# Bebra777228/PolGen-RVC

Measured on AMD Instinct MI355X. Metric: real-time-factor (audio-sec/wall-sec) per GPU, 30s@16kHz RMVPE->48kHz, higher is better.
Workload: dtype f32 (conv products as 3 fp16 MFMAs of a hi/lo split, fp32 accumulate; fp32 elsewhere)

## Files before the change

### include/rvcx.h

```cpp
#ifndef RVCX_H
#define RVCX_H
#include <stdint.h>

#ifdef __cplusplus
extern "C" {
#endif

typedef struct rvcx_ctx rvcx_ctx;

typedef struct {
  const char* name;
  const void* data;
  int32_t dtype;
  int32_t ndim;
  int64_t shape[4];
} rvcx_tensor;

typedef struct {
  int32_t inter_channels, hidden_channels, filter_channels, n_heads, n_layers, kernel_size;
  int32_t n_resblocks;
  int32_t res_kernels[4];
  int32_t res_dilations[4][3];
  int32_t n_ups;
  int32_t up_rates[6], up_kernels[6];
// ... 359 lines not shown
int rvcx_debug_inject(rvcx_ctx*, int what);
double rvcx_flop_counter(rvcx_ctx*, int reset);
void* rvcx_stream(rvcx_ctx*);

int rvcx_op_fcpe_post(rvcx_ctx*, const float* raw_hd, int F_in, int p_len, double pitch, double f0_min, double f0_max,
                      int32_t* coarse, float* f0);
int rvcx_op_conv1d(rvcx_ctx*, const float* x, const float* w, const float* bias, const float* res,
                   float* y, int B, int Cin, int Tin, int Cout, int K, int stride, int dil,
                   int pad_left, int Tout, int groups, int pre_lrelu, float pre_slope, int act,
                   float act_slope, const int32_t* lens_in, const int32_t* lens_out);
int rvcx_op_resblock_pair(rvcx_ctx*, const float* x, const float* w1, const float* b1, const float* w2,
                          const float* b2, float* y, int B, int C, int T, int K, int dil, float slope, int fused,
                          const int32_t* lens);
int rvcx_op_resblock3(rvcx_ctx*, const float* x, const float* w1, const float* b1, const float* w2, const float* b2,
                      float* y, int B, int C, int T, const int32_t* dils, float slope, const int32_t* lens);
int rvcx_bench_resblock_pair(rvcx_ctx*, int B, int C, int T, int K, int dil, int fused, int iters,
                             float* ms_per_launch);
int rvcx_bench_conv1d(rvcx_ctx*, int B, int Cin, int Tin, int Cout, int K, int stride, int dil, int groups,
                      int iters, float* ms_per_launch);
int rvcx_conv_override(int tile, int variant, int splitk);
int rvcx_fx_stretch_override(int chunk_frames, int segment_frames);
int rvcx_op_convtranspose1d(rvcx_ctx*, const float* x, const float* w, const float* bias, float* y,
                            int B, int Cin, int Tin, int Cout, int K, int stride, int pad,
                            int pre_lrelu, float pre_slope);
int rvcx_op_conv2d3x3(rvcx_ctx*, const float* x, const float* w, const float* bias, const float* res,
                      float* y, int B, int Cin, int H, int W, int Cout, int act);
int rvcx_op_convblock2d(rvcx_ctx*, const float* x, const float* w1, const float* b1, const float* w2, const float* b2,
                        const float* wsc, const float* bsc, float* y, int B, int Cin, int Cout, int H, int W,
                        const int32_t* rows);
int rvcx_op_convtranspose2d(rvcx_ctx*, const float* x, const float* w, const float* bias, float* y,
// ... 44 lines not shown
```

### polgen-rvc_amd/_lib.py

```python
from __future__ import annotations

import ctypes as C
import os
import threading
import types
from typing import Optional, Sequence

import numpy as np

_HERE = os.path.dirname(os.path.abspath(__file__))
LIB_PATH = os.environ.get("RVCX_LIBRARY") or os.path.join(_HERE, "librvcx.so")


class RvcxError(RuntimeError):
    pass


class Tensor(C.Structure):
    _fields_ = [("name", C.c_char_p), ("data", C.c_void_p), ("dtype", C.c_int32),
                ("ndim", C.c_int32), ("shape", C.c_int64 * 4)]


class SynthCfg(C.Structure):
    _fields_ = [("inter_channels", C.c_int32), ("hidden_channels", C.c_int32),
# ... 98 lines not shown
    k = min(Lx, Lb)
    fin = np.sin(0.5 * np.pi * np.arange(Lx) / max(Lx - 1, 1)) ** 2
    out[:k] = y[d:d + k] * fin[:k] + b[:k] * (1.0 - fin[:k])
    return out, y[d + Lb:d + Lb + Lx].copy(), d, scores, mags


_lib = None

SYMBOLS = [
    "rvcx_create", "rvcx_destroy", "rvcx_last_error", "rvcx_version", "rvcx_load_hubert",
    "rvcx_load_rmvpe", "rvcx_index_exhaustive", "rvcx_load_crepe", "rvcx_crepe_frames", "rvcx_crepe_predict", "rvcx_op_crepe_decode", "rvcx_get_f0_crepe_x", "rvcx_load_fcpe", "rvcx_fcpe_f0", "rvcx_fcpe_frames", "rvcx_get_f0_fcpe_x", "rvcx_op_fcpe_post", "rvcx_load_synth", "rvcx_unload_synth", "rvcx_load_index", "rvcx_load_index_ivf",
    "rvcx_weights_regions", "rvcx_weights_adopt", "rvcx_weights_clone", "rvcx_rmvpe_f0", "rvcx_rmvpe_frames", "rvcx_rmvpe_mel", "rvcx_synth_infer_taps", "rvcx_hubert_features",
    "rvcx_hubert_frames", "rvcx_synth_infer", "rvcx_synth_infer_window", "rvcx_synth_dec_rf", "rvcx_synth_upp", "rvcx_index_blend",
    "rvcx_out_len", "rvcx_convert_batch", "rvcx_convert_batch_f64", "rvcx_micro_batch", "rvcx_bucket_length", "rvcx_last_micro_batches", "rvcx_last_cuts", "rvcx_noise_len",
    "rvcx_get_f0", "rvcx_get_f0_x", "rvcx_vc", "rvcx_vc_frames", "rvcx_last_timing",
    "rvcx_flop_counter", "rvcx_fp32_reruns", "rvcx_mem_info", "rvcx_conv_profile", "rvcx_conv_profile_csv", "rvcx_stream", "rvcx_op_conv1d", "rvcx_op_resblock_pair", "rvcx_bench_resblock_pair", "rvcx_bench_conv1d", "rvcx_conv_override", "rvcx_op_convtranspose1d",
    "rvcx_op_conv2d3x3", "rvcx_op_convblock2d", "rvcx_op_convtranspose2d", "rvcx_op_attention", "rvcx_op_layernorm_c",
    "rvcx_op_bigru", "rvcx_op_highpass", "rvcx_highpass_exact", "rvcx_convert_batch_ex", "rvcx_get_f0_x_ex", "rvcx_fp32_layers", "rvcx_fp32_pinned",
    "rvcx_gru_fallbacks", "rvcx_gru_publish_probe", "rvcx_debug_inject", "rvcx_f0_file_track", "rvcx_op_gemm_tm", "rvcx_op_layernorm_tm",
    "rvcx_resample_len", "rvcx_resample_f64", "rvcx_resample_f64_kind", "rvcx_bench_gemm", "rvcx_device_info",
    "rvcx_convert_submit", "rvcx_convert_wait", "rvcx_convert_poll", "rvcx_convert_inflight", "rvcx_ticket_lead_ms",
    "rvcx_synth_infer_head", "rvcx_op_sola", "rvcx_stream_open", "rvcx_stream_step", "rvcx_stream_reset", "rvcx_stream_close",
    "rvcx_stream_out_len", "rvcx_stream_noise_len", "rvcx_stream_frames",
    "rvcx_stream_open_io", "rvcx_stream_in_len", "rvcx_stream_delays", "rvcx_stream_resample_delay", "rvcx_stream_last_taps",
    "rvcx_stream_set", "rvcx_op_stream_resample",
    "rvcx_stream_open_fx", "rvcx_stream_out_channels", "rvcx_stream_set_fx", "rvcx_stream_last_fx_ms", "rvcx_op_stream_fx",
    "rvcx_fx_reverb_host",
    "rvcx_fx_chain", "rvcx_op_fx_highpass", "rvcx_op_fx_compressor", "rvcx_op_fx_gate", "rvcx_op_fx_reverb", "rvcx_op_fx_shelf",
    "rvcx_op_fx_chorus", "rvcx_op_fx_mix", "rvcx_fx_chunk", "rvcx_fx_last_passes", "rvcx_fx_cte", "rvcx_fx_delay",
    "rvcx_fx_coeffs", "rvcx_fx_highpass_host", "rvcx_fx_biquad_host", "rvcx_fx_follower_host", "rvcx_fx_compressor_host",
    "rvcx_fx_gate_host", "rvcx_fx_comb_host", "rvcx_fx_allpass_host", "rvcx_fx_chorus_host", "rvcx_fx_mix_host",
# ... 1006 lines not shown
        return y

    def resblock_pair(self, x, w1, b1, w2, b2, dil=1, slope=0.1, fused=True, lens=None):
        x, w1, w2 = f32(x), f32(w1), f32(w2)
        B, Cc, T = x.shape
        K = w1.shape[2]
        y = np.empty_like(x)
        b1 = None if b1 is None else f32(b1)
        b2 = None if b2 is None else f32(b2)
        li = i32(lens)
        self._ck(lib().rvcx_op_resblock_pair(self._h, _p(x), _p(w1), _p(b1), _p(w2), _p(b2), _p(y), B, Cc, T, K, dil,
                                             C.c_float(slope), 1 if fused else 0, _p(li, C.c_int32)),
                 "op_resblock_pair")
        return y

    def resblock3(self, x, w1, b1, w2, b2, dils=(1, 3, 5), slope=0.1, lens=None):
        x, w1, w2 = f32(x), f32(w1), f32(w2)
        B, Cc, T = x.shape
        y = np.empty_like(x)
        b1 = None if b1 is None else f32(b1)
        b2 = None if b2 is None else f32(b2)
        d = i32(list(dils))
        li = i32(lens)
        self._ck(lib().rvcx_op_resblock3(self._h, _p(x), _p(w1), _p(b1), _p(w2), _p(b2), _p(y), B, Cc, T, _p(d, C.c_int32),
                                         C.c_float(slope), _p(li, C.c_int32)), "op_resblock3")
        return y

    def bench_resblock_pair(self, B, Cc, T, K, dil=1, fused=True, iters=10):
        ms = C.c_float(0)
        self._ck(lib().rvcx_bench_resblock_pair(self._h, B, Cc, T, K, dil, 1 if fused else 0, iters, C.byref(ms)),
# ... 1088 lines not shown
```

### polgen-rvc_amd/csrc/api_ops.hip

```cpp
#include "api_internal.h"
#include "h3_device.h"

using namespace rvcx;
using namespace rvcx::api;

static void to_host(Ctx& c, float* h, const float* d, size_t n) {
  RVCX_HIP(hipMemcpyAsync(h, d, n * sizeof(float), hipMemcpyDeviceToHost, c.stream));
  RVCX_HIP(hipStreamSynchronize(c.stream));
}
#define TEMP_REGION(C) WeightRegion tmp_region_; RegionScope tmp_scope_(*(C), tmp_region_)

extern "C" {

int rvcx_op_conv1d(rvcx_ctx* ctx, const float* x, const float* w, const float* bias, const float* res,
                   float* y, int B, int Cin, int Tin, int Cout, int K, int stride, int dil,
                   int pad_left, int Tout, int groups, int pre_lrelu, float pre_slope, int act,
                   float act_slope, const int32_t* lens_in, const int32_t* lens_out) {
  API_BEGIN(ctx)
  TEMP_REGION(C);
  size_t nx = (size_t)B * Cin * Tin, ny = (size_t)B * Cout * Tout;
  C->arena.reserve((nx + 2 * ny) * 4 + (64 << 20));
  C->arena.reset();
  ConvW L = make_conv(*C, w, bias, Cout, Cin / groups, K, groups, true);
  float* dx = to_dev(*C, x, nx);
// ... 211 lines not shown
  RVCX_HIP(hipEventCreate(&e0));
  RVCX_HIP(hipEventCreate(&e1));
  RVCX_HIP(hipEventRecord(e0, C->stream));
  for (int i = 0; i < iters; ++i) once();
  RVCX_HIP(hipEventRecord(e1, C->stream));
  RVCX_HIP(hipEventSynchronize(e1));
  float ms = 0.f;
  RVCX_HIP(hipEventElapsedTime(&ms, e0, e1));
  *ms_per_launch = ms / iters;
  (void)hipEventDestroy(e0);
  (void)hipEventDestroy(e1);
  C->arena.reset();
  API_END
}

int rvcx_conv_override(int tile, int variant, int splitk) {
  REQUIRE_DEBUG(nullptr, "rvcx_conv_override")
  rvcx::g_conv_override.tile = tile;
  rvcx::g_conv_override.variant = variant;
  rvcx::g_conv_override.splitk = splitk;
  return 0;
}

int rvcx_bench_conv1d(rvcx_ctx* ctx, int B, int Cin, int Tin, int Cout, int K, int stride, int dil, int groups,
                      int iters, float* ms_per_launch) {
  REQUIRE_DEBUG(ctx, "rvcx_bench_conv1d")
  API_BEGIN(ctx)
  TEMP_REGION(C);
  const int pad = (K * dil - dil) / 2;
  const int Tout = (Tin + 2 * pad - dil * (K - 1) - 1) / stride + 1;
// ... 660 lines not shown
```

### polgen-rvc_amd/csrc/conv.h

```cpp
#pragma once
#include "common.h"

namespace rvcx {

enum Act { ACT_NONE = 0, ACT_LRELU = 1, ACT_RELU = 2, ACT_GELU = 3, ACT_TANH = 4, ACT_SIGMOID = 5 };
enum OutMode { OUT_NORMAL = 0, OUT_SHUF1D = 1, OUT_SHUF2D = 2, OUT_TRANSPOSED = 3 };
enum Acc2 { ACC2_NONE = 0, ACC2_SET = 1, ACC2_ADD = 2, ACC2_ADD_DIV = 3 };

struct ConvArgs {
  const float* x = nullptr;
  const float* w = nullptr;
  const void* w_h3 = nullptr;
  const void* x_split = nullptr;
  void* y_split = nullptr;
  const float* bias = nullptr;
  const float* res = nullptr;
  float* y = nullptr;
  float* y2 = nullptr;
  const int* lens_in = nullptr;
  const int* lens_out = nullptr;
  int B = 1;
  int Cin_g = 0, Cin_gp = 0, Cout_g = 0, Cout_gp = 0, groups = 1;
  int Tin = 0;
  int Nout = 0;
// ... 117 lines not shown
bool convt_thin_ok(const ConvArgs& a);
void launch_convt_thin(const ConvArgs& a, hipStream_t stream);
void convt_thin_init();
constexpr int kConvtThinSlot = 61;
bool conv3_thin_ok(const ConvArgs& a);
void launch_conv3_thin(const ConvArgs& a, hipStream_t stream);
constexpr int kConv3ThinSlot = 59;
bool conv_deep_ok(const ConvArgs& a);
void launch_conv_deep(const ConvArgs& a, hipStream_t stream);
constexpr int kConvDeepSlot = 63;
bool conv_h3_enabled();
bool conv_h3_configured();
bool conv_h3_split_ok(const ConvArgs& a);
void launch_splitk_finish(const ConvArgs& a, hipStream_t stream);
void conv_h3_describe(ConvProfile* p);
struct ConvOverride { int tile = -1, variant = -1, splitk = -1; };
extern ConvOverride g_conv_override;
void conv_fast_init();
double conv_flops(const ConvArgs& a);

int conv_cin_pad(int cin_g);
int conv_cout_pad(int cout_g);
std::vector<float> pack_conv_weight(const float* w, int cout, int cin_g, int k, int groups);
struct PolyPhase1d {
  std::vector<float> w;
  std::vector<float> bias;
  int taps = 0;
  int pad = 0;
  int cout_total = 0;
};
// ... 5 lines not shown
```

### polgen-rvc_amd/csrc/conv_h3.hip

```cpp
#include <algorithm>
#include <cmath>
#include <cstdlib>

#include "conv.h"
#include "conv_device.h"
#include "h3_device.h"

#ifdef RVCX_ABLATION
#define H3_DBG(a, bit) ((a).dbg & (bit))
#else
#define H3_DBG(a, bit) 0
#endif

namespace rvcx {

template <int BM, int BN, int WR, int WC, int KKT, int HALO, int STRIDE, bool LIN, bool XS = false>
__global__ __launch_bounds__(256, ((LIN && BM * BN >= 8192) || BN >= 512) ? 2 : 3) void conv_h3_kernel(const ConvArgs a) {
  constexpr int WM = BM / (32 * WR), WN = BN / (32 * WC);
  constexpr int WROW = LIN ? BN : BN * STRIDE + HALO;
  constexpr int NBTILE = LIN ? KKT : 1;
  constexpr int A_ELEMS = KKT * 2 * 2 * BM;
  constexpr int NA = (A_ELEMS + 255) / 256;
  constexpr int B_TASKS = NBTILE * 2 * WROW;
  constexpr int NBT = (B_TASKS + 255) / 256;
// ... 310 lines not shown
  if (a.groups != 1 || a.ksize == 1 || a.out_mode != OUT_NORMAL) return false;
  if (a.stride != 1 && !(a.stride == 2 && a.kw == a.ksize)) return false;
  if (a.Cin_g % 16 != 0 || a.Cout_g % 16 != 0 || a.Cin_g != a.Cin_gp) return false;
  {
    int lo = 1 << 30, hi = -(1 << 30);
    for (int kk = 0; kk < a.ksize; ++kk) {
      lo = std::min(lo, conv_tap_off(a, kk));
      hi = std::max(hi, conv_tap_off(a, kk));
    }
    if (hi - lo > 320) return false;
  }
  if ((long)a.Cin_gp * a.x_cs * 4 >= kH3Oob || (long)a.Cout_g * a.y_cs * 4 >= kH3Oob) return false;
  return true;
}

int launch_conv_h3(ConvArgs& a, int halo, int off_min, hipStream_t stream) {
  const bool split = a.x_split || a.y_split;
  RVCX_CHECK(!split || conv_h3_split_ok(a), "conv_h3: pre-split activations on a launch that cannot take them");
  if (!a.w_h3 || !conv_h3_enabled()) return -1;
  if (a.Cin_gp % 16 != 0 || (a.stride != 1 && !(a.stride == 2 && a.kw == a.ksize))) return -1;
  if (a.groups != 1 && (split || a.ksize == 1 || a.stride != 1 || a.out_mode != OUT_NORMAL || a.Cin_g != a.Cin_gp)) return -1;
  if ((long)a.Cin_gp * a.x_cs * 4 >= kH3Oob || (long)a.ksize * a.Cin_gp * a.Cout_gp * 4 >= kH3Oob) return -1;
  const bool lin = a.ksize == 1 && a.stride == 1;
  const int nchunk = a.Cin_gp / 16;
  const long cap_item = a.part_cap_item > 0 ? a.part_cap_item : a.part_cap;
  static const bool wide3x3 = getenv("RVCX_WIDE3X3") && atoi(getenv("RVCX_WIDE3X3")) != 0;
  auto select = [&](int Bsel, int forcedS, int* tile_out, int* s_out) {
    int best = -1, S = 1;
    double best_t = 1e300;
    for (int t = 0; t < kNumH3; ++t) {
      const H3Cfg& F = kH3[t];
      if (g_conv_override.tile >= 100 && g_conv_override.tile - 100 != t) continue;
      if (F.lin != lin || F.stride != a.stride) continue;
// ... 22 lines not shown
    *tile_out = best;
    *s_out = S;
  };
  int best = -1, S = 1;
  select(1, 0, &best, &S);
  static const int tile2_mask = getenv("RVCX_TILE2_MASK") ? atoi(getenv("RVCX_TILE2_MASK")) : 255;
  const int cls = (a.out_mode != OUT_NORMAL) ? 8 : (lin ? 2 : (halo > 64 ? 1 : 4));
  int cls2 = cls;
  if (a.x_split || a.y_split) cls2 |= 16;
  const bool tile_for_batch = (tile2_mask & cls) && (!(cls2 & 16) || (tile2_mask & 16));
  if (best >= 0 && a.B > 1 && tile_for_batch) {
    int b2 = -1, s2 = 1;
    select(a.B, S, &b2, &s2);
    if (b2 >= 0 && s2 == S) best = b2;
  }
  if (best < 0) return -1;
  const H3Cfg& F = kH3[best];
  a.off_min = off_min;
  a.wrow = halo;
  a.splitk = S;
  {
    static int dbg = -1;
    if (dbg < 0) dbg = getenv("RVCX_CONV_DBG") ? atoi(getenv("RVCX_CONV_DBG")) : 0;
    a.dbg = dbg;
  }
  dim3 grid(cdiv(a.Nout, F.bn), cdiv(a.Cout_gp, F.bm), a.B * a.groups * S);
  {
    static const bool log = getenv("RVCX_CONV_LOG") != nullptr;
    if (log)
      fprintf(stderr, "h3 tile %d (%dx%d halo %d) S %d grid %u %u %u B %d Cin %d Cout %d k %d Nout %d xs %d ys %d\n", best,
              F.bm, F.bn, F.halo, S, grid.x, grid.y, grid.z, a.B, a.Cin_g, a.Cout_g, a.ksize, a.Nout, a.x_split != nullptr,
              a.y_split != nullptr);
  }
  hipLaunchKernelGGL(a.x_split ? F.kern_xs : F.kern, grid, dim3(256), 0, stream, a);
  if (S > 1) launch_splitk_finish(a, stream);
  RVCX_HIP(hipGetLastError());
  return h3_slot(best);
}

}
```

### polgen-rvc_amd/csrc/ctx.h

```cpp
#pragma once
#include <memory>

#include "common.h"
#include "conv.h"
#include "gemm.h"

namespace rvcx {

struct SynthModel;
struct RmvpeModel;
struct FcpeModel;
struct CrepeModel;
struct HubertModel;
struct IndexData;

class WeightRegion {
 public:
  static constexpr size_t kChunkBytes = (size_t)32 << 20;
  static constexpr int kMaxFlags = 4096;
  static constexpr size_t kHeaderBytes = kMaxFlags;
  WeightRegion() {
    flags_.reset(new uint8_t[kMaxFlags]);
    std::memset(flags_.get(), 0, kMaxFlags);
  }
// ... 224 lines not shown
  }
  void gemm_on(GemmArgs a, hipStream_t s) {
    const double f = 2.0 * (double)a.rows * a.cout * a.cin;
    flops += f;
    a.ovf = dev_err;
    a.seq = ++launch_seq;
    {
      const int si = (s == stream2) ? 1 : (s == aux[0] ? 2 : (s == aux[1] ? 3 : 0));
      if (!splitk_buf[si]) RVCX_HIP(hipMalloc(&splitk_buf[si], kSplitKFloats * splitk_items * sizeof(float)));
      a.part = splitk_buf[si];
      a.part_cap = kSplitKFloats * splitk_items;
    }
    conv_launch_gemm(a, f, s);
  }
  void conv(const ConvArgs& a) { conv_on(a, stream); }
  void conv_on(ConvArgs a, hipStream_t s) {
    flops += conv_flops(a);
    const int si = (s == stream2) ? 1 : (s == aux[0] ? 2 : (s == aux[1] ? 3 : 0));
    if (!splitk_buf[si]) RVCX_HIP(hipMalloc(&splitk_buf[si], kSplitKFloats * splitk_items * sizeof(float)));
    a.part = splitk_buf[si];
    a.part_cap = kSplitKFloats * splitk_items;
    a.part_cap_item = kSplitKFloats;
    a.ovf = dev_err;
    a.seq = ++launch_seq;
    launch_conv(a, s);
  }
};

struct RegionScope {
  Ctx& c;
  WeightRegion* prev;
  RegionScope(Ctx& cc, WeightRegion& r) : c(cc), prev(cc.slab.cur_) { cc.slab.cur_ = &r; }
  ~RegionScope() { c.slab.cur_ = prev; }
};

struct ConvW {
  const float* w = nullptr;
// ... 56 lines not shown
```

### polgen-rvc_amd/csrc/layers.h

```cpp
#pragma once
#include "ctx.h"

namespace rvcx {

inline ConvArgs conv1d_args(const ConvW& w, const float* x, float* y, int B, int Tin, int Tout,
                            int stride = 1, int dil = 1, int pad = 0) {
  ConvArgs a;
  conv_set_weights(a, w);
  a.x = x;
  a.y = y;
  a.B = B;
  a.Tin = Tin;
  a.Nout = Tout;
  a.stride = stride;
  a.dil = dil;
  a.pad = pad;
  a.x_bs = (long)w.cin * Tin;
  a.x_cs = Tin;
  a.y_bs = (long)w.cout * Tout;
  a.y_cs = Tout;
  return a;
}

inline void conv_set_res(ConvArgs& a, const float* res, int C, int T) {
  a.res = res;
  a.res_bs = (long)C * T;
  a.res_cs = T;
}

struct ConvT1dW {
  ConvW w;
  int stride = 1, pad_t = 0, cout_real = 0, k_orig = 0, taps_pad = 0;
};

inline ConvArgs convT1d_args(const ConvT1dW& L, const float* x, float* y, int B, int Tin, int Tout) {
  ConvArgs a;
  conv_set_weights(a, L.w);
  a.x = x;
  a.y = y;
  a.B = B;
  a.Tin = Tin;
  a.Nout = cdiv(Tout + L.pad_t, L.stride);
  a.stride = 1;
// ... 76 lines not shown
```

### polgen-rvc_amd/csrc/ops.hip

```cpp
#include <algorithm>
#include <cmath>
#include <vector>

#include "conv.h"
#include "h3_device.h"
#include "ops.h"

namespace rvcx {

__device__ __forceinline__ float wave_sum(float v) {
#pragma unroll
  for (int o = 32; o > 0; o >>= 1) v += __shfl_xor(v, o);
  return v;
}

__device__ __forceinline__ float gelu_erf(float v) {
  return 0.5f * v * (1.f + erff(v * 0.70710678118654752440f));
}

constexpr int LN_TX = 16, LN_PARTS = 16, LN_MAXC = 1024, LN_RPT = LN_MAXC / LN_PARTS;
__global__ __launch_bounds__(256) void layernorm_c_kernel(const float* __restrict__ x,
                                                          const float* __restrict__ gamma,
                                                          const float* __restrict__ beta, float* __restrict__ y,
                                                          int C, int T, float eps, const int* lens) {
// ... 475 lines not shown
}
void launch_flip_channels(const float* x, float* y, int B, int C, int T, hipStream_t s) {
  long n = (long)B * C * T;
  hipLaunchKernelGGL(flip_channels_kernel, EW_GRID(n), 0, s, x, y, C, T, n);
}

__global__ void wn_gate_kernel(const float* a, const float* g, int goff, int gstride, float* acts, int H, int T,
                               long total) {
  for (long idx = blockIdx.x * 256L + threadIdx.x; idx < total; idx += (long)gridDim.x * 256) {
    const int t = idx % T;
    const long bc = idx / T;
    const int c = bc % H;
    const long b = bc / H;
    const float ta = a[(b * 2 * H + c) * T + t] + g[b * gstride + goff + c];
    const float sa = a[(b * 2 * H + H + c) * T + t] + g[b * gstride + goff + H + c];
    acts[idx] = tanhf(ta) * (1.f / (1.f + expf(-sa)));
  }
}
void launch_wn_gate(const float* a, const float* g, int goff, int gstride, float* acts, int B, int H, int T,
                    hipStream_t s) {
  long n = (long)B * H * T;
  hipLaunchKernelGGL(wn_gate_kernel, EW_GRID(n), 0, s, a, g, goff, gstride, acts, H, T, n);
}

__global__ void wn_res_skip_kernel(float* x, float* out, const float* rs, int H, int T, int last, int first,
                                   const int* lens, long total) {
  for (long idx = blockIdx.x * 256L + threadIdx.x; idx < total; idx += (long)gridDim.x * 256) {
    const int t = idx % T;
    const long bc = idx / T;
    const int c = bc % H;
    const long b = bc / H;
// ... 472 lines not shown
```

### polgen-rvc_amd/csrc/synth.hip

```cpp
#include <algorithm>
#include <cmath>
#include <cstdlib>

#include "models.h"
#include "ops.h"

namespace rvcx {

std::vector<float> wn_weight(const TensorTable& t, const std::string& p, int dim) {
  if (t.has(p + ".weight")) return t.f32(p + ".weight");
  std::string gn = p + ".parametrizations.weight.original0", vn = p + ".parametrizations.weight.original1";
  if (!t.has(gn)) {
    gn = p + ".weight_g";
    vn = p + ".weight_v";
  }
  std::vector<float> g = t.f32(gn), v = t.f32(vn);
  const auto shp = t.shape(vn);
  RVCX_CHECK(shp.size() == 3, "weight-norm tensor must be 3-D: " + p);
  const int64_t d0 = shp[0], d1 = shp[1], d2 = shp[2];
  std::vector<float> w(v.size());
  if (dim == 0) {
    RVCX_CHECK((int64_t)g.size() == d0, "weight_g shape: " + p);
    for (int64_t a = 0; a < d0; ++a) {
      double ss = 0.0;
// ... 312 lines not shown

  float* z = A.alloc<float>((size_t)B * inter * T);
  float* z2 = A.alloc<float>((size_t)B * inter * T);
  launch_sample_z(stats, io.z_noise, z, B, inter, T, lens, s);
  if (head > 0) {
    launch_copy_strided(z + head, z2, B * inter, Tk, T, Tk, s);
    std::swap(z, z2);
  }
  float* g = A.alloc<float>((size_t)B * gin);
  for (int b = 0; b < B; ++b)
    RVCX_HIP(hipMemcpyAsync(g + (size_t)b * gin, m.emb_g + (size_t)sidv[b] * gin, gin * sizeof(float),
                            hipMemcpyDeviceToDevice, s));
  {
    float* h = att;
    float* xin = qkv;
    float* acts = tmp;
    float* rs = hbuf;
    RVCX_CHECK(filt >= 2 * hid, "buffer reuse assumes filter_channels >= 2*hidden");
    float* wout = A.alloc<float>((size_t)B * hid * T);
    float* mbuf = A.alloc<float>((size_t)B * half * T);
    float* gc = A.alloc<float>((size_t)B * 6 * hid);
    for (int f = 3; f >= 0; --f) {
      const auto& F = m.flows[f];
      launch_flip_channels(z, z2, B, inter, Tk, s);
      std::swap(z, z2);
      ConvArgs a = conv1d_args(F.pre, z, h, B, Tk, Tk);
      a.x_bs = (long)inter * Tk;
      a.lens_out = lens;
      c.conv(a);
      a = conv1d_args(F.cond, g, gc, B, 1, 1);
      c.conv(a);
      for (int i = 0; i < 3; ++i) {
        a = conv1d_args(F.in_l[i], h, xin, B, Tk, Tk, 1, 1, (F.in_l[i].k - 1) / 2);
        a.lens_in = lens;
        a.lens_out = lens;
        c.conv(a);
        launch_wn_gate(xin, gc, i * 2 * hid, 6 * hid, acts, B, hid, Tk, s);
        a = conv1d_args(F.rs_l[i], acts, rs, B, Tk, Tk);
        a.lens_out = lens;
        c.conv(a);
        launch_wn_res_skip(h, wout, rs, B, hid, Tk, i == 2, i == 0, lens, s);
      }
      a = conv1d_args(F.post, wout, mbuf, B, Tk, Tk);
      a.lens_out = lens;
      c.conv(a);
      launch_coupling_sub(z, mbuf, B, half, Tk, lens, s);
    }
  }
  if (io.z_out)
    RVCX_HIP(hipMemcpyAsync(io.z_out, z, (size_t)B * inter * Tk * sizeof(float), hipMemcpyDeviceToDevice, s));
  tm.mark(2);
  if (io.ev_decoder) RVCX_HIP(hipEventRecord(io.ev_decoder, s));

  if (!c.serial) RVCX_HIP(hipStreamWaitEvent(s, c.ev_src[1], 0));
  static const int dec_batch_env = getenv("RVCX_DEC_BATCH") ? std::max(1, atoi(getenv("RVCX_DEC_BATCH"))) : 8;
  bool equal_lens = true;
// ... 207 lines not shown
```

Measured before the change: 1224.

## Fuse WaveNet flow layer into a single MFMA kernel

Adds a fused kernel for each WaveNet layer in the flow. It runs the K=5 input conv, the tanh·sigmoid gate, the 1x1 res/skip conv and the residual/skip accumulation in one launch, keeping the gated activations in shared memory as hi/lo fp16 splits. This replaces four launches per layer and the global-memory round-trips for xin, acts and rs. The cost is a specialized kernel limited to hid=192 and K=5, split-k handled by in-register folding, and a fallback to the old path for any other shape.

```diff
diff --git a/include/rvcx.h b/include/rvcx.h
--- a/include/rvcx.h
+++ b/include/rvcx.h
@@ -397,6 +397,10 @@
                           const int32_t* lens);
 int rvcx_op_resblock3(rvcx_ctx*, const float* x, const float* w1, const float* b1, const float* w2, const float* b2,
                       float* y, int B, int C, int T, const int32_t* dils, float slope, const int32_t* lens);
+int rvcx_op_wn_layer(rvcx_ctx*, const float* h, const float* wout, const float* gc, const float* w_in, const float* b_in,
+                     const float* w_rs, const float* b_rs, float* h_out, float* wout_out, int B, int hid, int T, int K, int goff,
+                     int gstride, int first, int last, int fused, const int32_t* lens);
+int rvcx_bench_wn_layer(rvcx_ctx*, int B, int T, int last, int fused, int iters, float* ms_per_layer);
 int rvcx_bench_resblock_pair(rvcx_ctx*, int B, int C, int T, int K, int dil, int fused, int iters,
                              float* ms_per_launch);
 int rvcx_bench_conv1d(rvcx_ctx*, int B, int Cin, int Tin, int Cout, int K, int stride, int dil, int groups,
diff --git a/polgen-rvc_amd/_lib.py b/polgen-rvc_amd/_lib.py
--- a/polgen-rvc_amd/_lib.py
+++ b/polgen-rvc_amd/_lib.py
@@ -136,7 +136,7 @@
     "rvcx_hubert_frames", "rvcx_synth_infer", "rvcx_synth_infer_window", "rvcx_synth_dec_rf", "rvcx_synth_upp", "rvcx_index_blend",
     "rvcx_out_len", "rvcx_convert_batch", "rvcx_convert_batch_f64", "rvcx_micro_batch", "rvcx_bucket_length", "rvcx_last_micro_batches", "rvcx_last_cuts", "rvcx_noise_len",
     "rvcx_get_f0", "rvcx_get_f0_x", "rvcx_vc", "rvcx_vc_frames", "rvcx_last_timing",
-    "rvcx_flop_counter", "rvcx_fp32_reruns", "rvcx_mem_info", "rvcx_conv_profile", "rvcx_conv_profile_csv", "rvcx_stream", "rvcx_op_conv1d", "rvcx_op_resblock_pair", "rvcx_bench_resblock_pair", "rvcx_bench_conv1d", "rvcx_conv_override", "rvcx_op_convtranspose1d",
+    "rvcx_flop_counter", "rvcx_fp32_reruns", "rvcx_mem_info", "rvcx_conv_profile", "rvcx_conv_profile_csv", "rvcx_stream", "rvcx_op_conv1d", "rvcx_op_resblock_pair", "rvcx_op_wn_layer", "rvcx_bench_wn_layer", "rvcx_bench_resblock_pair", "rvcx_bench_conv1d", "rvcx_conv_override", "rvcx_op_convtranspose1d",
     "rvcx_op_conv2d3x3", "rvcx_op_convblock2d", "rvcx_op_convtranspose2d", "rvcx_op_attention", "rvcx_op_layernorm_c",
     "rvcx_op_bigru", "rvcx_op_highpass", "rvcx_highpass_exact", "rvcx_convert_batch_ex", "rvcx_get_f0_x_ex", "rvcx_fp32_layers", "rvcx_fp32_pinned",
     "rvcx_gru_fallbacks", "rvcx_gru_publish_probe", "rvcx_debug_inject", "rvcx_f0_file_track", "rvcx_op_gemm_tm", "rvcx_op_layernorm_tm",
@@ -1173,6 +1173,24 @@
                  "op_resblock_pair")
         return y
 
+    def wn_layer(self, h, wout, gc, w_in, b_in, w_rs, b_rs, goff=0, first=False, last=False, fused=True, lens=None):
+        h, gc, w_in, w_rs, b_in, b_rs = f32(h), f32(gc), f32(w_in), f32(w_rs), f32(b_in), f32(b_rs)
+        B, hid, T = h.shape
+        wout = np.zeros_like(h) if wout is None else f32(wout)
+        h_out, wout_out = np.empty_like(h), np.empty_like(h)
+        li = i32(lens)
+        self._ck(lib().rvcx_op_wn_layer(self._h, _p(h), _p(wout), _p(gc), _p(w_in), _p(b_in), _p(w_rs), _p(b_rs),
+                                        _p(h_out), _p(wout_out), B, hid, T, w_in.shape[2], goff, gc.shape[1],
+                                        1 if first else 0, 1 if last else 0, 1 if fused else 0, _p(li, C.c_int32)),
+                 "op_wn_layer")
+        return h_out, wout_out
+
+    def bench_wn_layer(self, B, T, last=False, fused=True, iters=20):
+        ms = C.c_float(0)
+        self._ck(lib().rvcx_bench_wn_layer(self._h, B, T, 1 if last else 0, 1 if fused else 0, iters, C.byref(ms)),
+                 "bench_wn_layer")
+        return ms.value
+
     def resblock3(self, x, w1, b1, w2, b2, dils=(1, 3, 5), slope=0.1, lens=None):
         x, w1, w2 = f32(x), f32(w1), f32(w2)
         B, Cc, T = x.shape
diff --git a/polgen-rvc_amd/csrc/api_ops.hip b/polgen-rvc_amd/csrc/api_ops.hip
--- a/polgen-rvc_amd/csrc/api_ops.hip
+++ b/polgen-rvc_amd/csrc/api_ops.hip
@@ -249,6 +249,91 @@
   API_END
 }
 
+int rvcx_op_wn_layer(rvcx_ctx* ctx, const float* h, const float* wout, const float* gc, const float* w_in, const float* b_in,
+                     const float* w_rs, const float* b_rs, float* h_out, float* wout_out, int B, int hid, int T, int K, int goff,
+                     int gstride, int first, int last, int fused, const int32_t* lens) {
+  API_BEGIN(ctx)
+  TEMP_REGION(C);
+  const size_t n = (size_t)B * hid * T;
+  C->arena.reserve(n * 4 * 8 + (64 << 20));
+  C->arena.reset();
+  ConvW Li = make_conv(*C, w_in, b_in, 2 * hid, hid, K, 1, true);
+  ConvW Lr = make_conv(*C, w_rs, b_rs, last ? hid : 2 * hid, hid, 1, 1, true);
+  float* dh = to_dev(*C, h, n);
+  float* dalt = C->arena.alloc<float>(n);
+  float* dw = C->arena.alloc<float>(n);
+  if (first) RVCX_HIP(hipMemsetAsync(dw, 0xff, n * 4, C->stream));
+  else RVCX_HIP(hipMemcpyAsync(dw, wout, n * 4, hipMemcpyDefault, C->stream));
+  RVCX_HIP(hipMemsetAsync(dalt, 0xff, n * 4, C->stream));
+  float* dxin = C->arena.alloc<float>(2 * n);
+  float* drs = C->arena.alloc<float>(2 * n);
+  WnStep st;
+  st.in_l = &Li;
+  st.rs_l = &Lr;
+  st.gc = to_dev(*C, gc, (size_t)B * gstride);
+  st.goff = goff;
+  st.gstride = gstride;
+  st.lens = (lens ? to_dev(*C, lens, B) : nullptr);
+  st.B = B;
+  st.hid = hid;
+  st.T = T;
+  st.first = first;
+  st.last = last;
+  const float* dres = wn_layer_on(*C, st, dh, dalt, dw, dxin, drs, (fused && !g_force_fp32) ? 1 : 0);
+  to_host(*C, h_out, dres, n);
+  to_host(*C, wout_out, dw, n);
+  C->arena.reset();
+  API_END
+}
+
+int rvcx_bench_wn_layer(rvcx_ctx* ctx, int B, int T, int last, int fused, int iters, float* ms_per_layer) {
+  REQUIRE_DEBUG(ctx, "rvcx_bench_wn_layer")
+  API_BEGIN(ctx)
+  TEMP_REGION(C);
+  const int hid = 192, K = 5;
+  const size_t n = (size_t)B * hid * T;
+  C->arena.reserve(n * 4 * 8 + (64 << 20));
+  C->arena.reset();
+  std::vector<float> wi((size_t)2 * hid * hid * K), wr((size_t)2 * hid * hid), bias((size_t)2 * hid, 0.05f), g((size_t)B * 2 * hid, 0.1f);
+  for (size_t i = 0; i < wi.size(); ++i) wi[i] = ((float)((i * 2654435761u) % 2001) / 1000.f - 1.f) / std::sqrt((float)hid * K);
+  for (size_t i = 0; i < wr.size(); ++i) wr[i] = ((float)((i * 2246822519u) % 2001) / 1000.f - 1.f) / (4.f * std::sqrt((float)hid));
+  ConvW Li = make_conv(*C, wi.data(), bias.data(), 2 * hid, hid, K, 1, true);
+  ConvW Lr = make_conv(*C, wr.data(), bias.data(), last ? hid : 2 * hid, hid, 1, 1, true);
+  float* dh = C->arena.alloc<float>(n);
+  float* dalt = C->arena.alloc<float>(n);
+  float* dw = C->arena.alloc<float>(n);
+  float* dxin = C->arena.alloc<float>(2 * n);
+  float* drs = C->arena.alloc<float>(2 * n);
+  launch_randn(dh, n, 1, 0, C->stream);
+  RVCX_HIP(hipMemsetAsync(dw, 0, n * 4, C->stream));
+  WnStep st;
+  st.in_l = &Li;
+  st.rs_l = &Lr;
+  st.gc = to_dev(*C, g.data(), g.size());
+  st.gstride = 2 * hid;
+  st.B = B;
+  st.hid = hid;
+  st.T = T;
+  st.last = last;
+  RVCX_HIP(hipStreamSynchronize(C->stream));
+  auto once = [&]() { (void)wn_layer_on(*C, st, dh, dalt, dw, dxin, drs, fused ? 1 : 0); };
+  once();
+  hipEvent_t e0, e1;
+  RVCX_HIP(hipEventCreate(&e0));
+  RVCX_HIP(hipEventCreate(&e1));
+  RVCX_HIP(hipEventRecord(e0, C->stream));
+  for (int i = 0; i < iters; ++i) once();
+  RVCX_HIP(hipEventRecord(e1, C->stream));
+  RVCX_HIP(hipEventSynchronize(e1));
+  float ms = 0.f;
+  RVCX_HIP(hipEventElapsedTime(&ms, e0, e1));
+  *ms_per_layer = ms / iters;
+  (void)hipEventDestroy(e0);
+  (void)hipEventDestroy(e1);
+  C->arena.reset();
+  API_END
+}
+
 int rvcx_conv_override(int tile, int variant, int splitk) {
   REQUIRE_DEBUG(nullptr, "rvcx_conv_override")
   rvcx::g_conv_override.tile = tile;
diff --git a/polgen-rvc_amd/csrc/conv.h b/polgen-rvc_amd/csrc/conv.h
--- a/polgen-rvc_amd/csrc/conv.h
+++ b/polgen-rvc_amd/csrc/conv.h
@@ -155,6 +155,29 @@
 bool conv_h3_split_ok(const ConvArgs& a);
 void launch_splitk_finish(const ConvArgs& a, hipStream_t stream);
 void conv_h3_describe(ConvProfile* p);
+int conv_h3_splitk(const ConvArgs& a);
+
+struct WnArgs {
+  const float* h = nullptr;
+  float* h_out = nullptr;
+  float* wout = nullptr;
+  const float* gc = nullptr;
+  int goff = 0, gstride = 0;
+  const void* w_in = nullptr;
+  const void* w_rs = nullptr;
+  const float* b_in = nullptr;
+  const float* b_rs = nullptr;
+  const int* lens = nullptr;
+  int B = 1, hid = 0, k = 0, T = 0;
+  int first = 0, last = 0;
+  int splitk = 1;
+  int* ovf = nullptr;
+  int* ovf_in = nullptr;
+  int* ovf_rs = nullptr;
+  int seq = 0;
+};
+bool wn_layer_ok(const WnArgs& a);
+void launch_wn_layer(const WnArgs& a, hipStream_t stream);
 struct ConvOverride { int tile = -1, variant = -1, splitk = -1; };
 extern ConvOverride g_conv_override;
 void conv_fast_init();
diff --git a/polgen-rvc_amd/csrc/conv_h3.hip b/polgen-rvc_amd/csrc/conv_h3.hip
--- a/polgen-rvc_amd/csrc/conv_h3.hip
+++ b/polgen-rvc_amd/csrc/conv_h3.hip
@@ -348,9 +348,8 @@
   return true;
 }
 
-int launch_conv_h3(ConvArgs& a, int halo, int off_min, hipStream_t stream) {
+static int h3_plan(const ConvArgs& a, int halo, int* s_out) {
   const bool split = a.x_split || a.y_split;
-  RVCX_CHECK(!split || conv_h3_split_ok(a), "conv_h3: pre-split activations on a launch that cannot take them");
   if (!a.w_h3 || !conv_h3_enabled()) return -1;
   if (a.Cin_gp % 16 != 0 || (a.stride != 1 && !(a.stride == 2 && a.kw == a.ksize))) return -1;
   if (a.groups != 1 && (split || a.ksize == 1 || a.stride != 1 || a.out_mode != OUT_NORMAL || a.Cin_g != a.Cin_gp)) return -1;
@@ -403,6 +402,15 @@
     select(a.B, S, &b2, &s2);
     if (b2 >= 0 && s2 == S) best = b2;
   }
+  *s_out = S;
+  return best;
+}
+
+int launch_conv_h3(ConvArgs& a, int halo, int off_min, hipStream_t stream) {
+  const bool split = a.x_split || a.y_split;
+  RVCX_CHECK(!split || conv_h3_split_ok(a), "conv_h3: pre-split activations on a launch that cannot take them");
+  int S = 1;
+  const int best = h3_plan(a, halo, &S);
   if (best < 0) return -1;
   const H3Cfg& F = kH3[best];
   a.off_min = off_min;
@@ -427,4 +435,16 @@
   return h3_slot(best);
 }
 
-}
+int conv_h3_splitk(const ConvArgs& a) {
+  if (a.stride != 1 || a.groups != 1 || a.out_mode != OUT_NORMAL || a.Cin_g == 1 || a.Cout_g == 1) return -1;
+  if (conv3_thin_ok(a) || conv_deep_ok(a)) return -1;
+  int lo = 1 << 30, hi = -(1 << 30);
+  for (int kk = 0; kk < a.ksize; ++kk) {
+    lo = std::min(lo, conv_tap_off(a, kk));
+    hi = std::max(hi, conv_tap_off(a, kk));
+  }
+  int S = 1;
+  return h3_plan(a, hi - lo, &S) < 0 ? -1 : S;
+}
+
+}
diff --git a/polgen-rvc_amd/csrc/ctx.h b/polgen-rvc_amd/csrc/ctx.h
--- a/polgen-rvc_amd/csrc/ctx.h
+++ b/polgen-rvc_amd/csrc/ctx.h
@@ -262,13 +262,16 @@
     conv_launch_gemm(a, f, s);
   }
   void conv(const ConvArgs& a) { conv_on(a, stream); }
-  void conv_on(ConvArgs a, hipStream_t s) {
-    flops += conv_flops(a);
+  void conv_scratch(ConvArgs& a, hipStream_t s) {
     const int si = (s == stream2) ? 1 : (s == aux[0] ? 2 : (s == aux[1] ? 3 : 0));
     if (!splitk_buf[si]) RVCX_HIP(hipMalloc(&splitk_buf[si], kSplitKFloats * splitk_items * sizeof(float)));
     a.part = splitk_buf[si];
     a.part_cap = kSplitKFloats * splitk_items;
     a.part_cap_item = kSplitKFloats;
+  }
+  void conv_on(ConvArgs a, hipStream_t s) {
+    flops += conv_flops(a);
+    conv_scratch(a, s);
     a.ovf = dev_err;
     a.seq = ++launch_seq;
     launch_conv(a, s);
diff --git a/polgen-rvc_amd/csrc/layers.h b/polgen-rvc_amd/csrc/layers.h
--- a/polgen-rvc_amd/csrc/layers.h
+++ b/polgen-rvc_amd/csrc/layers.h
@@ -27,6 +27,17 @@
   a.res_bs = (long)C * T;
   a.res_cs = T;
 }
+
+struct WnStep {
+  const ConvW* in_l = nullptr;
+  const ConvW* rs_l = nullptr;
+  const float* gc = nullptr;
+  int goff = 0, gstride = 0;
+  const int* lens = nullptr;
+  int B = 1, hid = 0, T = 0;
+  int first = 0, last = 0;
+};
+float* wn_layer_on(Ctx& c, const WnStep& st, float* h, float* h_alt, float* wout, float* xin, float* rs, int mode = -1);
 
 struct ConvT1dW {
   ConvW w;
diff --git a/polgen-rvc_amd/csrc/ops.hip b/polgen-rvc_amd/csrc/ops.hip
--- a/polgen-rvc_amd/csrc/ops.hip
+++ b/polgen-rvc_amd/csrc/ops.hip
@@ -5,6 +5,7 @@
 #include "conv.h"
 #include "h3_device.h"
 #include "ops.h"
+#include "wn_device.h"
 
 namespace rvcx {
 
@@ -513,7 +514,7 @@
     const long b = bc / H;
     const float ta = a[(b * 2 * H + c) * T + t] + g[b * gstride + goff + c];
     const float sa = a[(b * 2 * H + H + c) * T + t] + g[b * gstride + goff + H + c];
-    acts[idx] = tanhf(ta) * (1.f / (1.f + expf(-sa)));
+    acts[idx] = wn_gate_act(ta, sa);
   }
 }
 void launch_wn_gate(const float* a, const float* g, int goff, int gstride, float* acts, int B, int H, int T,
diff --git a/polgen-rvc_amd/csrc/synth.hip b/polgen-rvc_amd/csrc/synth.hip
--- a/polgen-rvc_amd/csrc/synth.hip
+++ b/polgen-rvc_amd/csrc/synth.hip
@@ -350,7 +350,7 @@
   {
     float* h = att;
     float* xin = qkv;
-    float* acts = tmp;
+    float* h_alt = tmp;
     float* rs = hbuf;
     RVCX_CHECK(filt >= 2 * hid, "buffer reuse assumes filter_channels >= 2*hidden");
     float* wout = A.alloc<float>((size_t)B * hid * T);
@@ -366,16 +366,22 @@
       c.conv(a);
       a = conv1d_args(F.cond, g, gc, B, 1, 1);
       c.conv(a);
+      float* hc = h;
+      float* ha = h_alt;
       for (int i = 0; i < 3; ++i) {
-        a = conv1d_args(F.in_l[i], h, xin, B, Tk, Tk, 1, 1, (F.in_l[i].k - 1) / 2);
-        a.lens_in = lens;
-        a.lens_out = lens;
-        c.conv(a);
-        launch_wn_gate(xin, gc, i * 2 * hid, 6 * hid, acts, B, hid, Tk, s);
-        a = conv1d_args(F.rs_l[i], acts, rs, B, Tk, Tk);
-        a.lens_out = lens;
-        c.conv(a);
-        launch_wn_res_skip(h, wout, rs, B, hid, Tk, i == 2, i == 0, lens, s);
+        WnStep st;
+        st.in_l = &F.in_l[i];
+        st.rs_l = &F.rs_l[i];
+        st.gc = gc;
+        st.goff = i * 2 * hid;
+        st.gstride = 6 * hid;
+        st.lens = lens;
+        st.B = B;
+        st.hid = hid;
+        st.T = Tk;
+        st.first = i == 0;
+        st.last = i == 2;
+        if (wn_layer_on(c, st, hc, ha, wout, xin, rs) != hc) std::swap(hc, ha);
       }
       a = conv1d_args(F.post, wout, mbuf, B, Tk, Tk);
       a.lens_out = lens;
diff --git a/polgen-rvc_amd/csrc/wn_device.h b/polgen-rvc_amd/csrc/wn_device.h
--- /dev/null
+++ b/polgen-rvc_amd/csrc/wn_device.h
@@ -0,0 +1,8 @@
+#pragma once
+#include "common.h"
+
+namespace rvcx {
+
+__device__ __forceinline__ float wn_gate_act(float ta, float sa) { return tanhf(ta) * (1.f / (1.f + expf(-sa))); }
+
+}
diff --git a/polgen-rvc_amd/csrc/wn_layer.hip b/polgen-rvc_amd/csrc/wn_layer.hip
--- /dev/null
+++ b/polgen-rvc_amd/csrc/wn_layer.hip
@@ -0,0 +1,326 @@
+#include <cstdlib>
+
+#include "conv.h"
+#include "conv_device.h"
+#include "h3_device.h"
+#include "layers.h"
+#include "ops.h"
+#include "wn_device.h"
+
+namespace rvcx {
+
+namespace {
+
+constexpr int kHid = 192, kTaps = 5, kPad = 2, kTS = 32;
+constexpr int kChunks = kHid / 16;
+constexpr int kRowH = kTS + 2 * kPad;
+constexpr int kWaves = 6, kThreads = 64 * kWaves;
+constexpr int kStepsIn = kChunks * kTaps;
+static_assert(kStepsIn % 4 == 0 && kChunks % 4 == 0, "the weight ring walks four k-steps per turn");
+
+struct WFrag {
+  uint4 hi[2], lo[2];
+};
+
+template <bool LAST>
+__global__ __launch_bounds__(kThreads) void wn_layer_kernel(const WnArgs a) {
+  constexpr int NT2 = LAST ? 1 : 2;
+  constexpr int CP_IN = 2 * kHid, CP_RS = LAST ? kHid : 2 * kHid;
+  constexpr float inv = 1.f / kH3Scale;
+  __shared__ uint4 Hs[kChunks * 4 * kRowH];
+  __shared__ uint4 Gs[kChunks * 4 * kTS];
+
+  const int tid = threadIdx.x, lane = tid & 63;
+  const int wave = __builtin_amdgcn_readfirstlane(tid >> 6);
+  const int i = lane & 31, h = lane >> 5;
+  const int b = blockIdx.z, t0 = blockIdx.x * kTS, T = a.T;
+  const int len_in = a.lens ? min(a.lens[b], T) : T;
+  const int len_out = a.lens ? a.lens[b] : 0x7fffffff;
+  const bool dead = t0 >= len_out;
+  const int nn = t0 + i;
+  const bool live = nn < len_out;
+  const int S = a.splitk;
+  const float* hb = a.h + (long)b * kHid * T;
+  const int cbase = 32 * wave + 4 * h;
+  bool ovf_h = false, ovf_a = false;
+
+  f32x16 acc[2], tot[2];
+#pragma unroll
+  for (int t = 0; t < 2; ++t)
+#pragma unroll
+    for (int r = 0; r < 16; ++r) {
+      acc[t][r] = 0.f;
+      tot[t][r] = 0.f;
+    }
+
+  if (!dead) {
+    const H3Rsrc wi = h3_rsrc(a.w_in, kTaps * kChunks * 4 * CP_IN * 16);
+    const H3Rsrc wr = h3_rsrc(a.w_rs, kChunks * 4 * CP_RS * 16);
+    int voff_in[2], voff_rs[2];
+#pragma unroll
+    for (int t = 0; t < 2; ++t) {
+      voff_in[t] = (h * CP_IN + (t * 6 + wave) * 32 + i) * 16;
+      voff_rs[t] = (h * CP_RS + (t * 6 + wave) * 32 + i) * 16;
+    }
+    auto load_in = [&](int s, WFrag& f) {
+      const int chunk = s / kTaps, tap = s - chunk * kTaps;
+      const int base = (tap * kChunks + chunk) * 4 * CP_IN * 16;
+#pragma unroll
+      for (int t = 0; t < 2; ++t) {
+        f.hi[t] = h3_load4s(wi, voff_in[t], base);
+        f.lo[t] = h3_load4s(wi, voff_in[t], base + 2 * CP_IN * 16);
+      }
+    };
+    auto load_rs = [&](int s, WFrag& f) {
+      const int base = s * 4 * CP_RS * 16;
+#pragma unroll
+      for (int t = 0; t < NT2; ++t) {
+        f.hi[t] = h3_load4s(wr, voff_rs[t], base);
+        f.lo[t] = h3_load4s(wr, voff_rs[t], base + 2 * CP_RS * 16);
+      }
+    };
+    WFrag f0, f1, f2, f3;
+    load_in(0, f0);
+    load_in(1, f1);
+    load_in(2, f2);
+    load_in(3, f3);
+
+    for (int t = tid; t < kChunks * 2 * kRowH; t += kThreads) {
+      const int ch2 = t / kRowH, p = t - ch2 * kRowH;
+      const int pos = t0 - kPad + p;
+      const bool ok = pos >= 0 && pos < len_in;
+      const float* src = hb + (long)(ch2 * 8) * T + pos;
+      half8 hi, lo;
+#pragma unroll
+      for (int q = 0; q < 8; ++q) {
+        const float v = ok ? src[(long)q * T] : 0.f;
+        ovf_h |= !(fabsf(v) < kH3ActLimit);
+        const _Float16 vh = (_Float16)v;
+        hi[q] = vh;
+        lo[q] = (_Float16)((v - (float)vh) * kH3Scale);
+      }
+      const int chunk = ch2 >> 1, hh = ch2 & 1;
+      Hs[(chunk * 4 + hh) * kRowH + p] = __builtin_bit_cast(uint4, hi);
+      Hs[(chunk * 4 + 2 + hh) * kRowH + p] = __builtin_bit_cast(uint4, lo);
+    }
+    __syncthreads();
+
+    auto fold = [&]() {
+#pragma unroll
+      for (int t = 0; t < 2; ++t)
+#pragma unroll
+        for (int r = 0; r < 16; ++r) {
+          const float p = acc[t][r] * inv;
+          tot[t][r] = S > 1 ? tot[t][r] + p : p;
+          acc[t][r] = 0.f;
+        }
+    };
+    auto step_in = [&](const WFrag& f, int s) {
+      const int chunk = s / kTaps, tap = s - chunk * kTaps;
+      if (tap == 0 && chunk > 0 && (chunk * S) % kChunks == 0) fold();
+      const uint4* Bt = Hs + chunk * 4 * kRowH + i + tap;
+      const half8 b0 = __builtin_bit_cast(half8, Bt[h * kRowH]), b1 = __builtin_bit_cast(half8, Bt[(2 + h) * kRowH]);
+#pragma unroll
+      for (int t = 0; t < 2; ++t) {
+        const half8 a0 = __builtin_bit_cast(half8, f.hi[t]), a2 = __builtin_bit_cast(half8, f.lo[t]);
+        const half8 a1 = a0 * (_Float16)(1.f / kH3Scale);
+        acc[t] = h3_mfma(a0, b0, acc[t]);
+        acc[t] = h3_mfma(a1, b1, acc[t]);
+        acc[t] = h3_mfma(a2, b0, acc[t]);
+      }
+    };
+    for (int s = 0; s < kStepsIn; s += 4) {
+      const bool more = s + 4 < kStepsIn;
+      step_in(f0, s);
+      if (more) load_in(s + 4, f0);
+      step_in(f1, s + 1);
+      if (more) load_in(s + 5, f1);
+      step_in(f2, s + 2);
+      if (more) load_in(s + 6, f2);
+      step_in(f3, s + 3);
+      if (more) load_in(s + 7, f3);
+    }
+    fold();
+    load_rs(0, f0);
+    load_rs(1, f1);
+    load_rs(2, f2);
+    load_rs(3, f3);
+
+    {
+      const float* g = a.gc + (long)b * a.gstride + a.goff;
+#pragma unroll
+      for (int gq = 0; gq < 4; ++gq) {
+        typedef _Float16 half4 __attribute__((ext_vector_type(4)));
+        half4 hi, lo;
+#pragma unroll
+        for (int q = 0; q < 4; ++q) {
+          const int r = 4 * gq + q, c = cbase + q + 8 * gq;
+          float xa = tot[0][r] + a.b_in[c], xs = tot[1][r] + a.b_in[kHid + c];
+          if (S == 1) {
+            xa += 0.f;
+            xs += 0.f;
+          }
+          xa = live ? xa : 0.f;
+          xs = live ? xs : 0.f;
+          float v = wn_gate_act(xa + g[c], xs + g[kHid + c]);
+          asm volatile("" : "+v"(v));
+          if (nn < T) ovf_a |= !(fabsf(v) < kH3ActLimit);
+          const _Float16 vh = (_Float16)v;
+          hi[q] = vh;
+          lo[q] = (_Float16)((v - (float)vh) * kH3Scale);
+        }
+        const int chunk = 2 * wave + (gq >> 1), hh = gq & 1;
+        char* e = reinterpret_cast<char*>(Gs);
+        *reinterpret_cast<half4*>(e + ((chunk * 4 + hh) * kTS + i) * 16 + 8 * h) = hi;
+        *reinterpret_cast<half4*>(e + ((chunk * 4 + 2 + hh) * kTS + i) * 16 + 8 * h) = lo;
+      }
+    }
+    __syncthreads();
+
+    auto step_rs = [&](const WFrag& f, int s) {
+      const uint4* Bt = Gs + s * 4 * kTS + i;
+      const half8 b0 = __builtin_bit_cast(half8, Bt[h * kTS]), b1 = __builtin_bit_cast(half8, Bt[(2 + h) * kTS]);
+#pragma unroll
+      for (int t = 0; t < NT2; ++t) {
+        const half8 a0 = __builtin_bit_cast(half8, f.hi[t]), a2 = __builtin_bit_cast(half8, f.lo[t]);
+        const half8 a1 = a0 * (_Float16)(1.f / kH3Scale);
+        acc[t] = h3_mfma(a0, b0, acc[t]);
+        acc[t] = h3_mfma(a1, b1, acc[t]);
+        acc[t] = h3_mfma(a2, b0, acc[t]);
+      }
+    };
+    for (int s = 0; s < kChunks; s += 4) {
+      const bool more = s + 4 < kChunks;
+      step_rs(f0, s);
+      if (more) load_rs(s + 4, f0);
+      step_rs(f1, s + 1);
+      if (more) load_rs(s + 5, f1);
+      step_rs(f2, s + 2);
+      if (more) load_rs(s + 6, f2);
+      step_rs(f3, s + 3);
+      if (more) load_rs(s + 7, f3);
+    }
+#pragma unroll
+    for (int t = 0; t < NT2; ++t)
+#pragma unroll
+      for (int r = 0; r < 16; ++r) acc[t][r] *= inv;
+  }
+
+  if (nn < T) {
+    const long col = (long)b * kHid * T + nn;
+#pragma unroll
+    for (int r0 = 0; r0 < 16; r0 += 8) {
+      float hv[8], ov[8];
+#pragma unroll
+      for (int q = 0; q < 8; ++q) {
+        const int r = r0 + q, c = cbase + (r & 3) + 8 * (r >> 2);
+        hv[q] = LAST ? 0.f : a.h[col + (long)c * T];
+        ov[q] = a.first ? 0.f : a.wout[col + (long)c * T];
+      }
+#pragma unroll
+      for (int q = 0; q < 8; ++q) {
+        const int r = r0 + q, c = cbase + (r & 3) + 8 * (r >> 2);
+        if constexpr (!LAST) {
+          float rr = acc[0][r] + a.b_rs[c], sk = acc[1][r] + a.b_rs[kHid + c];
+          rr += 0.f;
+          sk += 0.f;
+          rr = live ? rr : 0.f;
+          sk = live ? sk : 0.f;
+          a.h_out[col + (long)c * T] = live ? (hv[q] + rr) : 0.f;
+          a.wout[col + (long)c * T] = a.first ? sk : ov[q] + sk;
+        } else {
+          float sk = acc[0][r] + a.b_rs[c];
+          sk += 0.f;
+          sk = live ? sk : 0.f;
+          const float o = a.first ? sk : ov[q] + sk;
+          a.wout[col + (long)c * T] = live ? o : 0.f;
+        }
+      }
+    }
+  }
+  if (ovf_h) report_h3_overflow(a.ovf, a.ovf_in, a.seq);
+  if (ovf_a) report_h3_overflow(a.ovf, a.ovf_rs, a.seq + 1);
+}
+
+}
+
+bool wn_layer_ok(const WnArgs& a) {
+  if (a.hid != kHid || a.k != kTaps || a.T <= 0 || a.B <= 0) return false;
+  if (!a.h || !a.wout || !a.gc || !a.w_in || !a.w_rs || !a.b_in || !a.b_rs) return false;
+  if (!a.last && (!a.h_out || a.h_out == a.h)) return false;
+  return a.splitk >= 1 && kChunks % a.splitk == 0;
+}
+
+void launch_wn_layer(const WnArgs& a, hipStream_t stream) {
+  RVCX_CHECK(wn_layer_ok(a), "wn layer: unsupported shape");
+  const dim3 grid(cdiv(a.T, kTS), 1, a.B);
+  if (a.last)
+    hipLaunchKernelGGL(wn_layer_kernel<true>, grid, dim3(kThreads), 0, stream, a);
+  else
+    hipLaunchKernelGGL(wn_layer_kernel<false>, grid, dim3(kThreads), 0, stream, a);
+  RVCX_HIP(hipGetLastError());
+}
+
+float* wn_layer_on(Ctx& c, const WnStep& st, float* h, float* h_alt, float* wout, float* xin, float* rs, int mode) {
+  static const bool env_on = !getenv("RVCX_WN_FUSE") || atoi(getenv("RVCX_WN_FUSE")) != 0;
+  const ConvW& Li = *st.in_l;
+  const ConvW& Lr = *st.rs_l;
+  const int B = st.B, hid = st.hid, T = st.T;
+  hipStream_t s = c.stream;
+  ConvArgs ai = conv1d_args(Li, h, xin, B, T, T, 1, 1, (Li.k - 1) / 2);
+  ai.lens_in = st.lens;
+  ai.lens_out = st.lens;
+  if (mode != 0 && (mode > 0 || env_on)) {
+    WnArgs a;
+    a.h = h;
+    a.h_out = st.last ? nullptr : h_alt;
+    a.wout = wout;
+    a.gc = st.gc;
+    a.goff = st.goff;
+    a.gstride = st.gstride;
+    a.lens = st.lens;
+    a.B = B;
+    a.hid = hid;
+    a.k = Li.k;
+    a.T = T;
+    a.first = st.first;
+    a.last = st.last;
+    const bool shape = Li.cin == hid && Li.cout == 2 * hid && Li.groups == 1 && Lr.k == 1 && Lr.cin == hid && Lr.groups == 1 &&
+                       Lr.cout == (st.last ? hid : 2 * hid) && Li.cout_gp == Li.cout && Lr.cout_gp == Lr.cout &&
+                       Li.cin_gp == hid && Lr.cin_gp == hid && Li.bias && Lr.bias;
+    if (shape && conv_h3_ok(Li) && conv_h3_ok(Lr)) {
+      ConvArgs plan = ai;
+      c.conv_scratch(plan, s);
+      a.splitk = conv_h3_splitk(plan);
+      ConvArgs ar = conv1d_args(Lr, h_alt, rs, B, T, T);
+      ar.lens_out = st.lens;
+      plan = ar;
+      c.conv_scratch(plan, s);
+      a.w_in = Li.w_h3;
+      a.w_rs = Lr.w_h3;
+      a.b_in = Li.bias;
+      a.b_rs = Lr.bias;
+      if (conv_h3_splitk(plan) == 1 && wn_layer_ok(a)) {
+        c.flops += conv_flops(ai) + conv_flops(ar);
+        a.ovf = c.dev_err;
+        a.ovf_in = Li.ovf_word;
+        a.ovf_rs = Lr.ovf_word;
+        a.seq = ++c.launch_seq;
+        ++c.launch_seq;
+        launch_wn_layer(a, s);
+        return st.last ? h : h_alt;
+      }
+    }
+    RVCX_CHECK(mode <= 0, "wn layer: shape not supported by the fused kernel");
+  }
+  float* acts = h_alt;
+  c.conv(ai);
+  launch_wn_gate(xin, st.gc, st.goff, st.gstride, acts, B, hid, T, s);
+  ConvArgs ar = conv1d_args(Lr, acts, rs, B, T, T);
+  ar.lens_out = st.lens;
+  c.conv(ar);
+  launch_wn_res_skip(h, wout, rs, B, hid, T, st.last, st.first, st.lens, s);
+  return h;
+}
+
+}
```

New measurement: 1232, median of 6. About the same (+0.7%).
